# KaranSankla/Lidar_Object_Detection

Measured on AMD Instinct MI355X. Metric: LiDAR points/sec projected+instance-labelled, higher is better.
Workload: dtype f64

## Files before the change

### lidar_object_detection_amd/_build.py

```python
import hashlib
import os
import shutil
import subprocess

_HERE = os.path.dirname(os.path.abspath(__file__))
CSRC = os.path.join(_HERE, "csrc")
LIB = os.path.join(_HERE, "liblpf.so")
LAB_LIB = os.path.join(_HERE, "liblpf_lab.so")
SOURCES = ("lpf_api.hip", "lpf_kernels.hip.h", "lpf_reader.hip.h", "lpf_wide.hip.h", "lpf_cams.hip.h", "lpf_cams_wide.hip.h",
           "lpf_frame_wide.hip.h", "lpf_depth_maps.hip.h", "lpf_depth_overlays.hip.h",
           "lpf_match2d.hip.h", "lpf_inside.hip.h", "lpf_box_points.hip.h", "lpf_box_views.hip.h", "lpf_assign.hip.h",
           "lpf_first_match.hip.h", "lpf_rle.hip.h")
ARCH = "gfx950"

FLAGS = ["--offload-arch=" + ARCH, "-O3", "-std=c++17", "-fPIC", "-shared", "-pthread", "-ldl",
         "-ffp-contract=off", "-fno-fast-math", "-Wall", "-Wno-unused-function"]


def hipcc():
    exe = shutil.which("hipcc") or "/opt/rocm/bin/hipcc"
    if not os.path.exists(exe):
        raise RuntimeError("hipcc not found (looked on PATH and in /opt/rocm/bin)")
    return exe


HEADER = os.path.join(os.path.dirname(_HERE), "include", "lpf.h")
_MARKER = b"LPF_BUILD_ID="


def source_id(lab=False):
    h = hashlib.sha256()
    for path in [os.path.join(CSRC, s) for s in SOURCES] + [HEADER]:
# ... 67 lines not shown
```

### lidar_object_detection_amd/csrc/lpf_api.hip

```cpp
#include "lpf_kernels.hip.h"
#include "lpf_wide.hip.h"
#include "lpf_cams.hip.h"
#include "lpf_cams_wide.hip.h"
#include "lpf_frame_wide.hip.h"
#include "lpf_depth_maps.hip.h"
#include "lpf_depth_overlays.hip.h"
#include "lpf_match2d.hip.h"
#include "lpf_assign.hip.h"
#include "lpf_inside.hip.h"
#include "lpf_box_points.hip.h"
#include "lpf_box_views.hip.h"
#include "lpf_first_match.hip.h"
#include "lpf_rle.hip.h"
#include "../../include/lpf.h"

#include <algorithm>
#include <cmath>
#include <cstdarg>
#include <cstdio>
#include <cstdlib>
#include <cstring>
#include <dlfcn.h>
#include <initializer_list>
#include <mutex>
// ... 258 lines not shown
    return fn(Flag<false>());
}

static_assert(LPF_RECT_FUSED_TILE == 1024, "LpfDirectRect tiles are instantiated for 1024 points only");
template <bool STEP, typename Fn> void with_tile_form(const TileSource &src, int rows, bool scan_tail, Fn &&fn)
{
    auto tail = [&](auto lt, auto rw) {
        if (STEP && scan_tail) fn(lt, rw, Flag<STEP>()); else fn(lt, rw, Flag<false>());
    };
    if (src.kind == TileSource::DIRECT_RECT) {
        if (!src.f32) fn(TypeTag<LpfDirectRect<uint8_t, 0>>(), Rows<4>(), Flag<false>());
        else fn(TypeTag<LpfDirectRect<float, 1>>(), Rows<4>(), Flag<false>());
    } else if (src.kind == TileSource::DIRECT) {
        with_rule(src.f32, src.rule, [&](auto kind) { tail(TypeTag<LpfDirect<typename decltype(kind)::elem, decltype(kind)::rule>>(), Rows<2>()); });
    } else {
        with_label(src.label_bytes, [&](auto lt) {
            if (rows == 2) tail(lt, Rows<2>());
            else if (STEP && rows == 8) tail(lt, Rows<STEP ? 8 : 4>());
            else tail(lt, Rows<4>());
        });
    }
}

hipError_t host_wait(lpf_ctx *c)
{
    ++c->stats[0];
    return hipStreamSynchronize(c->stream);
}

void launch_tail(hipStream_t st, const LpfParams &P, int ntail, bool pre)
{
    if (pre) hipLaunchKernelGGL((lpf_tail_t<true>), dim3((unsigned)ntail), dim3(LPF_BLOCK), 0, st, P);
    else hipLaunchKernelGGL((lpf_tail_t<false>), dim3((unsigned)ntail), dim3(LPF_BLOCK), 0, st, P);
}

void box_job_camera(LpfBoxJob &J, const double K[9], int W, int H)
{
    memcpy(J.K, K, sizeof J.K);
    J.W = W; J.H = H;
}

int box_job_blocks(const lpf_ctx::BoxSet &B) { return B.F * B.job.chunks; }

int launch_box_job(lpf_ctx *c, lpf_ctx::BoxSet &B, const double K[9], int W, int H)
{
    if (!B.take_job()) return LPF_OK;
// ... 45 lines not shown
    if (ride) {
        const lpf_ctx::Unpacked &U = c->masks.unpacked;
        J.masks = (const uint8_t *)U.masks; J.label = U.label; J.M = U.M; J.hw = (long long)c->H * c->W;
        J.rects = U.rects; J.W = c->W;
        J.total16 = (long long)U.F * (J.hw / 16);
        Y.npack = (int)((J.total16 + LPF_BLOCK - 1) / LPF_BLOCK);
    }
    const int nk1_pad = (Y.nk1 + 7) & ~7;
    Y.nper = (Y.ntail + 7) / 8;
    Y.kper = Y.nk1 > 0 ? 8 : 0;
    if (Y.nper > 0 && Y.nk1 > 0) {
        const long long k = ((long long)nk1_pad * LPF_TAIL_SPREAD_20THS / 20 / 8) / Y.nper;
        Y.kper = (int)(k < 1 ? 1 : k) * 8;
    }
    const long long rest = (long long)nk1_pad - (long long)Y.nper * Y.kper;
    Y.rest = (int)(rest > 0 ? rest : 0);
    const long long grid = (long long)Y.nfin8 + Y.nbox8 + Y.nrg8 + (long long)Y.nper * (Y.kper + 8) + Y.rest + Y.npack;
    if (grid > 0) {
        const dim3 gs((unsigned)grid);
        ++c->stats[3];
        if (boxes) ++c->stats[5];
        with_tile_form<true>(tiles, KP.tile_pts >> 8, Q.valid && Q.pre, [&](auto lt, auto rw, auto pr) {
            with_flag(boxes, [&](auto bx) {
                hipLaunchKernelGGL((lpf_step_t<decltype(rw)::value, LPF_K1_FLAGS, typename decltype(lt)::type, decltype(pr)::value, decltype(bx)::value>),
                                   gs, dim3(LPF_BLOCK), 0, c->stream, KP, QP, RP, Y, J, XJ, GJ);
            });
        });
        LPF_HIP(c, hipGetLastError());
    }
    if (after) LPF_HIP(c, hipEventRecord(after, c->stream));
    if (KK.valid && KK.pre && KK.P.nseg_total > 0) {
        hipLaunchKernelGGL(lpf_scan_segments, dim3(KK.P.F), dim3(LPF_BLOCK), 0, c->stream, KK.P);
        LPF_HIP(c, hipGetLastError());
    }
    return LPF_OK;
}

lpf_ctx::Pending pending_run(const LpfParams &P, bool pre, int ntail, int nk1, const TileSource &src)
{
    return lpf_ctx::Pending{true, P, pre, ntail, nk1, src};
}

int queue_step(lpf_ctx *c, const lpf_ctx::Pending *cur, lpf_ctx::BoxSet *XB, hipEvent_t after, const LpfRectJob *RG)
{
    lpf_ctx::Pipeline &PL = c->pipe;
    const bool wait = cur && PL.defer;
    const lpf_ctx::Pending K = (cur && !wait) ? *cur : PL.k1, Q = PL.tail, R = PL.fin;
    int rc_ = launch_step(c, K, Q, R, cur ? &cur->src : nullptr, XB, after, RG);
// ... 545 lines not shown
}

int pack_unpacked(lpf_ctx *c)
{
    lpf_ctx::Masks &MK = c->masks;
    const lpf_ctx::Unpacked &U = MK.unpacked;
    if (!U.valid) return LPF_OK;
    lpf_ctx::Scratch &S = c->sc[MK.set];
    void *cur = nullptr;
    int rc = pack_masks(c, S.label_a, S.label_b, c->W, c->H, c->stream, U.masks, U.f32, U.rule, MK.bytes, U.F, U.M, 0, &cur, U.rects);
    if (rc) return rc;
    MK.packed(MK.F, MK.M, cur, MK.bytes);
    MK.forget_unpacked();
    return LPF_OK;
}

int plan_tile_source(lpf_ctx *c, bool fused, bool small, bool sparse_frames, int M, TileSource &src)
{
    src = TileSource();
    int rc;
    const lpf_ctx::Masks &MK = c->masks;
    const lpf_ctx::Unpacked &U = MK.unpacked;
    const bool readable = U.valid && U.pipelined == fused && M > 0 && sparse_frames;
    if (readable && !small && U.rects && ((!U.f32 && U.rule == 0) || (U.f32 && U.rule == 1))) src.kind = TileSource::DIRECT_RECT;
    else if (readable && small) src.kind = TileSource::DIRECT;
    else {
        src.ride_pack = U.valid && U.pipelined && fused && U.can_ride && M > 0;
        if (!src.ride_pack && (rc = pack_unpacked(c))) return rc;
        if (M > 0) src.kind = TileSource::PACKED;
    }
    if (M > 0 && fused && MK.set != c->pipe.run_set(fused))
        return fail(c, LPF_ERR_STATE, "the masks were set for another scratch set: in the pipelined modes the label images rotate with the scratch sets -- call lpf_set_masks_* before every lpf_run* (and after switching modes)");
    if (src.reads_masks()) {
        src.f32 = U.f32; src.rule = U.rule; src.img = U.masks;
        src.rects = U.rects;
    } else if (M > 0) {
        src.img = MK.img;
    }
    if (M > 0 && !src.img) return fail(c, LPF_ERR_STATE, "no masks for this run's scratch set: in the pipelined modes the label images rotate with the scratch sets -- call lpf_set_masks_* before every lpf_run* (and after switching modes)");
    src.label_bytes = (M > 0) ? MK.bytes : 4;
    return LPF_OK;
}


int check_frames(lpf_ctx *c, const char *who, const float *pts, const int64_t *frame_off, int F, int64_t slack)
{
    if (frame_off[0] != 0) return fail(c, LPF_ERR_ARG, "%s: frame_off[0] must be 0", who);
// ... 35 lines not shown
            if ((rc = reserve(c, dr, (size_t)F * m.M * 16))) return rc;
            LPF_HIP(c, hipMemcpyAsync(dr.p, m.rects, (size_t)F * m.M * 16, hipMemcpyHostToDevice, c->stream));
            d_rects = (const int32_t *)dr.p;
        }
        *host_in = true;
    }
    *masks = d_masks;
    *rects = rects_hold(m) ? (const int4 *)d_rects : nullptr;
    return LPF_OK;
}

struct Cam {
    const double *T, *K;
    double dmin, dmax;
    int W, H;
};
Cam ctx_cam(const lpf_ctx *c) { return Cam{c->T, c->K, c->dmin, c->dmax, c->W, c->H}; }
Cam input_cam(const lpf_cam_input &I) { return Cam{I.T_velo_to_rect, I.K, I.depth_min_excl, I.depth_max_excl, I.W, I.H}; }
void set_cam(LpfCam &P, const Cam &k)
{
    memcpy(P.T, k.T, sizeof P.T);
    memcpy(P.K, k.K, sizeof P.K);
    P.dmin = k.dmin; P.dmax = k.dmax; P.W = k.W; P.H = k.H;
}

struct NarrowLayout {
    int F = 0;
    bool small = false;
    int64_t seg_pts = 0;
    int nseg_total = 0, ngrp_total = 0, max_ngrp = 0;
    int nblk = 0;
    int nwblk = 0;
    int csplit = 1, ncblk = 0;
    bool few = false;
    bool pre_scan = false;
    int nseg_cap() const { return nseg_total > 0 ? nseg_total : 1; }
    int ngrp_cap() const { return ngrp_total > 0 ? ngrp_total : 1; }
    void split(int parts) { csplit = parts; ncblk = nwblk * parts; }
};

void narrow_layout(lpf_ctx *c, const int64_t *frame_off, int F, const lpf_ctx::BoxSet &BX, long long inst_cap, bool small, NarrowLayout &L)
{
    L = NarrowLayout();
    L.F = F; L.small = small;
    L.seg_pts = small ? LPF_SEG_SMALL : LPF_SEG_QUANTUM;
    c->h_frames.resize(F);
// ... 719 lines not shown
            LPF_HIP(c, hipEventCreate(&b));
            c->ev.push_back(a); c->ev.push_back(b);
        }
        e0 = c->ev[2 * c->ev_used]; e1 = c->ev[2 * c->ev_used + 1];
        ++c->ev_used;
        LPF_HIP(c, hipEventRecord(e0, c->stream));
    }
    if (fused) {
        const lpf_ctx::Pending cur = pending_run(P, L.pre_scan, ntail, nk1, src);
        if ((rc = queue_step(c, &cur, &BX, e1, (rect_tiles && tiles_wait) ? &RG : nullptr))) return rc;
        c->masks.forget_unpacked();
        c->pipe.parity = (c->pipe.parity + 1) % c->pipe.sets();
        return LPF_OK;
    }
    if (BX.job_ready() && nk1 > 0) {
        const lpf_ctx::Pending cur = pending_run(P, false, 0, nk1, src);
        lpf_ctx::Pending none;
        if ((rc = launch_step(c, cur, none, none, nullptr, &BX, e1))) return rc;
    } else {
    if ((rc = launch_box_job(c, BX))) return rc;
    if (nk1 > 0) {
        const dim3 g1((unsigned)nk1);
        with_tile_form<false>(src, P.tile_pts >> 8, false, [&](auto lt, auto rw, auto) {
            hipLaunchKernelGGL((lpf_k1_project_t<decltype(rw)::value, LPF_K1_FLAGS, typename decltype(lt)::type>), g1, dim3(LPF_BLOCK), 0, c->stream, P);
        });
        LPF_HIP(c, hipGetLastError());
        if (e1) LPF_HIP(c, hipEventRecord(e1, c->stream));
    }
    }
    if (L.pre_scan && L.nseg_total > 0) {
        hipLaunchKernelGGL(lpf_scan_segments, dim3(F), dim3(LPF_BLOCK), 0, c->stream, P);
        LPF_HIP(c, hipGetLastError());
    }
    if (ntail > 0) {
        if (small && P.count_boxes && c->geometry != 4 && (L.nblk <= LPF_WIDE_BELOW || c->geometry == 1)) {
            if (L.pre_scan) hipLaunchKernelGGL((lpf_tail_wide_t<true>), dim3((unsigned)ntail), dim3(64 * LPF_WIDE_WAVES), 0, c->stream, P);
            else hipLaunchKernelGGL((lpf_tail_wide_t<false>), dim3((unsigned)ntail), dim3(64 * LPF_WIDE_WAVES), 0, c->stream, P);
        } else {
            launch_tail(c->stream, P, ntail, L.pre_scan);
        }
        LPF_HIP(c, hipGetLastError());
    }
    hipLaunchKernelGGL(lpf_finalize, dim3(F), dim3(LPF_BLOCK), 0, c->stream, P);
    LPF_HIP(c, hipGetLastError());

    if (host_io) {
        std::vector<lpf_frame_summary> hs((size_t)F);
// ... 1626 lines not shown
```

### lidar_object_detection_amd/csrc/lpf_cams.hip.h

```cpp
#pragma once
#include "lpf_kernels.hip.h"

#define LPF_MAX_CAMS_DEV 4

struct LpfCamsArgs {
    LpfParams P[LPF_MAX_CAMS_DEV];
    int C;
    int ntail[LPF_MAX_CAMS_DEV];
};
static_assert(sizeof(LpfCamsArgs) <= 4096, "a kernel's argument segment holds 4 KB");

template <int ROWS, typename LT>
__global__ __launch_bounds__(LPF_BLOCK) void lpf_cams_stream(const LpfCamsArgs A)
{
    __shared__ unsigned s_cnt[LPF_MAX_CAMS_DEV][LPF_TAB_ROWS];
    float4 p[ROWS];
    lpf_k1_tile<ROWS, LPF_K1_FLAGS, LT, false>(A.P[0], (int)blockIdx.x, s_cnt[0], p);
    for (int cam = 1; cam < A.C; ++cam)
        lpf_k1_tile<ROWS, LPF_K1_FLAGS, LT, true>(A.P[cam], (int)blockIdx.x, s_cnt[cam], p);
}

template <bool PRE>
__global__ __launch_bounds__(LPF_BLOCK, 7) void lpf_cams_tail(const LpfCamsArgs A)
{
    __shared__ __attribute__((aligned(16))) char s_raw[LPF_TAIL_LDS];
    const int cam = (int)blockIdx.y;
    if ((int)blockIdx.x >= A.ntail[cam]) return;
    lpf_tail_block<PRE, 1>(A.P[cam], (int)blockIdx.x, s_raw);
}

__global__ __launch_bounds__(LPF_BLOCK) void lpf_cams_finalize(const LpfCamsArgs A)
{
    __shared__ unsigned s_tot[LPF_TAB_ROWS], s_c[LPF_FIN_STAGE];
    const LpfParams &P = A.P[blockIdx.y];
    const int f = (int)blockIdx.x;
    const LpfFrame fr = lpf_frame_record(P.frame0, P.frames, P.F > 1, f);
    lpf_finalize_frame(P, fr, f, s_tot, s_c);
}
```

### lidar_object_detection_amd/csrc/lpf_kernels.hip.h

```cpp
#pragma once
#include <hip/hip_runtime.h>
#include <stdint.h>

#define LPF_BLOCK 256
#define LPF_SEG_QUANTUM 4096
#define LPF_SEG_SMALL 1024
#define LPF_GROUP_SEGS 64
#define LPF_FRM_SHARDS 8
#define LPF_MAX_MASKS_DEV 32
#define LPF_TAB_ROWS 36
#define LPF_TAB_GROUPS 9

struct LpfFrame {
    long long pt_off;
    long long inst_base;
    int N;
    int seg_off;
    int nseg;
    int box_off;
    int B;
    int pad;
    long long cand_off;
    int cand_words;
    int grp_off;
    int shift;
    int pad4;
};

struct LpfCam {
    double T[12];
    double K[9];
    double dmin, dmax;
    int W, H;
};

struct LpfParams : LpfCam {
    int F, M;
    int seg_pts;
    int nseg_total;
    int nseg_cap;
    int ngrp_cap;
    int oriented;
    long long inst_cap;
    LpfFrame frame0;
    const LpfFrame *frames;
    const LpfFrame *segs;
    const int2 *blks;
    const int4 *cblks;
    int nblk, ncblk;
    int lists_small;
    int csplit;
    const float4 *pts;
    const void *label_img;
    const int4 *rects;
    const uint32_t *rect_grid;
    int rg_cw, rg_cells;
    const double *boxp;
    const float *boxq;
    const unsigned long long *cand;
    int2 *uv;
    uint32_t *label_bits;
    double *depth, *uf, *vf;
    long long *valid_idx;
    int2 *uv_valid;
    uint32_t *label_valid;
    long long *inst_idx;
    int32_t *count_out;
    void *summary;
    unsigned long long *vbal, *mbal;
    uint4 *seg_tab;
    uint4 *grp_tab;
    uint4 *frm_tab;
    uint4 *seg_pre;
    unsigned *cnt;
    float4 *mlist;
    int count_boxes;
    int count_lazy;
    int tile_pts;
};
static_assert(sizeof(LpfCam) == 192 && sizeof(LpfParams) == 576, "the camera leads LpfParams; neither layout may move");

__device__ __forceinline__ int lpf_lane() { return threadIdx.x & 63; }
__device__ __forceinline__ int lpf_wave() { return threadIdx.x >> 6; }

__device__ __forceinline__ int lpf_xcd_remap(int b, int n)
{
    const int q = n >> 3, r = n & 7, x = b & 7, i = b >> 3;
    return (x < r ? x * (q + 1) : r * (q + 1) + (x - r) * q) + i;
}

__device__ __forceinline__ int lpf_uni(int v) { return __builtin_amdgcn_readfirstlane(v); }
__device__ __forceinline__ long long lpf_uni64(long long v)
{
    return (long long)(((unsigned long long)(unsigned)lpf_uni((int)((unsigned long long)v >> 32)) << 32) | (unsigned)lpf_uni((int)v));
}
__device__ __forceinline__ LpfFrame lpf_frame_record(const LpfFrame &by_value, const LpfFrame *table, const bool many, const int idx)
{
    LpfFrame fr = by_value;
    if (many) {
        const LpfFrame t = table[lpf_uni(idx)];
        fr.pt_off = lpf_uni64(t.pt_off); fr.inst_base = lpf_uni64(t.inst_base); fr.N = lpf_uni(t.N); fr.seg_off = lpf_uni(t.seg_off);
        fr.nseg = lpf_uni(t.nseg); fr.box_off = lpf_uni(t.box_off); fr.B = lpf_uni(t.B); fr.pad = lpf_uni(t.pad);
        fr.cand_off = lpf_uni64(t.cand_off); fr.cand_words = lpf_uni(t.cand_words); fr.grp_off = lpf_uni(t.grp_off); fr.shift = lpf_uni(t.shift);
    }
    return fr;
}

__device__ __forceinline__ int32_t lpf_sat_i32(double r)
{
    int v;
    asm("v_cvt_i32_f64 %0, %1" : "=v"(v) : "v"(r));
    return (r != r) ? INT32_MIN : v;
}

__device__ __forceinline__ unsigned lpf_expo(double x) { return ((unsigned)__double2hiint(x) >> 20) & 0x7ffu; }

__device__ __forceinline__ void lpf_div2(double qx, double qy, double ad, double &uf, double &vf)
{
    const unsigned ea = lpf_expo(ad), ex = lpf_expo(qx), ey = lpf_expo(qy);
    const unsigned lo = min(ea, min(ex, ey)), hi = max(ea, max(ex, ey));
    if (lo >= 723u && hi <= 1323u) {
        double r = __builtin_amdgcn_rcp(ad);
        double e = fma(-ad, r, 1.0); r = fma(r, e, r);
        e = fma(-ad, r, 1.0);        r = fma(r, e, r);
        double q = qx * r; double s = fma(-ad, q, qx); uf = fma(s, r, q);
        q = qy * r;        s = fma(-ad, q, qy);        vf = fma(s, r, q);
    } else {
        uf = qx / ad;
        vf = qy / ad;
    }
}

__device__ __forceinline__ void lpf_project_point(const LpfCam &P, float fx, float fy, float fz,
                                                  double &uf, double &vf, double &d)
{
    const double x = (double)fx, y = (double)fy, z = (double)fz;
    double cx = P.T[0] * x; cx = fma(P.T[1], y, cx); cx = fma(P.T[2],  z, cx); cx = cx + P.T[3];
    double cy = P.T[4] * x; cy = fma(P.T[5], y, cy); cy = fma(P.T[6],  z, cy); cy = cy + P.T[7];
    double cz = P.T[8] * x; cz = fma(P.T[9], y, cz); cz = fma(P.T[10], z, cz); cz = cz + P.T[11];
    double qx = P.K[0] * cx; qx = fma(P.K[1], cy, qx); qx = fma(P.K[2], cz, qx);
    double qy = P.K[3] * cx; qy = fma(P.K[4], cy, qy); qy = fma(P.K[5], cz, qy);
    d = P.K[6] * cx; d = fma(P.K[7], cy, d); d = fma(P.K[8], cz, d);
    if (d == 0.0) d = -1e-6;
    lpf_div2(qx, qy, fabs(d), uf, vf);
}

__device__ __forceinline__ bool lpf_in_view(const LpfCam &P, int ui, int vi, double d)
{
    return ((unsigned)ui < (unsigned)P.W) && ((unsigned)vi < (unsigned)P.H) && (d > P.dmin) && (d < P.dmax);
}

__device__ __forceinline__ bool lpf_pixel(const LpfCam &P, double uf, double vf, double d, int &ui, int &vi)
{
    ui = lpf_sat_i32(rint(uf));
    vi = lpf_sat_i32(rint(vf));
    return lpf_in_view(P, ui, vi, d);
}

__device__ __forceinline__ unsigned lpf_f32_to_u8(float v)
{
    int t;
    if (!(v > -2147483904.0f && v < 2147483648.0f)) t = INT32_MIN; else t = (int)v;
    return (unsigned)t & 0xFFu;
}

template <typename T, int MODE>
__device__ __forceinline__ bool lpf_member(T v)
{
    if (MODE == 0) return v != 0;
    if (MODE == 1) return lpf_f32_to_u8((float)v) != 0u;
    if (MODE == 3) return (float)v > 0.5f;
    return lpf_f32_to_u8((float)v * 255.0f) == 255u;
}

template <typename T, int MODE> struct LpfDirect { };
template <typename LT> struct LpfIsDirect { static constexpr bool value = false; };
template <typename T, int MODE> struct LpfIsDirect<LpfDirect<T, MODE> > { static constexpr bool value = true; };

template <typename T, int MODE> struct LpfDirectRect { };
// ... 34 lines not shown
        }
        return l;
    }
    static __device__ __forceinline__ size_t frame_stride(const LpfParams &P) { return (size_t)P.M * (size_t)P.W * (size_t)P.H; }
};

template <typename T, int MODE>
struct LpfLabelSrc<LpfDirectRect<T, MODE> > {
    typedef T elem;
    static constexpr int mode = MODE;
    static __device__ __forceinline__ uint32_t get(const elem *__restrict__, const LpfParams &, const int, const int4 *, int, int) { return 0u; }
    static __device__ __forceinline__ size_t frame_stride(const LpfParams &P) { return (size_t)P.M * (size_t)P.W * (size_t)P.H; }
};

#define LPF_F_X4 1u
#define LPF_F_NTLOAD 2u
#define LPF_F_NTSTORE 4u
#define LPF_F_LAB_NOMATH 8u
#define LPF_F_LAB_NOGATHER 16u
#define LPF_F_LAB_NOSTORE 32u

#define LPF_F_LAB_NOBAL 64u
#define LPF_F_LAB_NOTAB 128u

#define LPF_RG_SHIFT 4
#define LPF_RG_CELL (1 << LPF_RG_SHIFT)
__device__ __forceinline__ unsigned lpf_wave_or(unsigned x);

template <int ROWS, unsigned FL, typename LT, bool PRELOADED>
__device__ __forceinline__ void lpf_k1_tile(const LpfParams &P, const int blk, unsigned *s_cnt, float4 (&p)[ROWS])
{
    constexpr int TILE = LPF_BLOCK * ROWS;
    static_assert(LPF_SEG_QUANTUM % TILE == 0 && (LPF_SEG_SMALL % TILE == 0 || ROWS >= 8), "tiles must divide segments (8-row and larger tiles: large geometry only)");
    const int tid = threadIdx.x, lane = lpf_lane(), wave = lpf_wave();
    const int tiles_per_seg = P.seg_pts / TILE;
    const int lb = lpf_xcd_remap(blk, P.nseg_total * tiles_per_seg);
    const int sid = lb / tiles_per_seg;
    LpfFrame fr = P.frame0;
    if (P.F > 1) fr = P.segs[__builtin_amdgcn_readfirstlane(sid)];
    const int f = fr.pad;
    const int sh = fr.shift;
    const long long pbase = fr.pt_off - sh;
    const int seg_start = (sid - fr.seg_off) * P.seg_pts;
    const int seg_end = min(seg_start + P.seg_pts, fr.N + sh);
    const int c = seg_start + (lb - sid * tiles_per_seg) * TILE;
    if (c >= seg_end) return;
    const float4 *__restrict__ pts = P.pts + pbase;
    typedef LpfLabelSrc<LT> Src;
    const typename Src::elem *__restrict__ limg =
        (P.label_img && P.M > 0) ? static_cast<const typename Src::elem *>(P.label_img) + (size_t)f * Src::frame_stride(P) : nullptr;
    const int rows_per_seg = P.seg_pts >> 6;
    if (tid < LPF_TAB_ROWS) s_cnt[tid] = 0;
    __syncthreads();
    unsigned nvalid_w = 0, nmask_w = 0;

    {
        const int wbase = c + wave * (ROWS * 64) + lane;
#pragma unroll
        for (int r = 0; r < ROWS; ++r) {
            if constexpr (PRELOADED) continue;
            const float4 *src = pts + min(wbase + r * 64, seg_end - 1);
            if (FL & LPF_F_NTLOAD) {
                typedef float f4v __attribute__((ext_vector_type(4)));
                const f4v t = __builtin_nontemporal_load(reinterpret_cast<const f4v *>(src));
                p[r] = make_float4(t.x, t.y, t.z, t.w);
            } else {
                p[r] = *src;
            }
        }
        uint32_t lab[ROWS];
        bool valid[ROWS];
        constexpr bool RECT = LpfIsDirectRect<LT>::value;
        const int4 *__restrict__ rc_f = ((RECT || LpfIsDirect<LT>::value) && P.rects) ? P.rects + (size_t)f * P.M : nullptr;
        const uint32_t *__restrict__ rgrid = (RECT && limg && P.rect_grid) ? P.rect_grid + (size_t)f * P.rg_cells : nullptr;
        const size_t mhw = (size_t)P.W * (size_t)P.H;
        unsigned long long myv = 0, mym = 0;
        auto consume = [&](const int r, uint32_t l, const bool okr) {
            const int idx = wbase + r * 64;
            if (idx >= sh && idx < seg_end && P.label_bits && !(FL & LPF_F_LAB_NOSTORE)) {
                if (FL & LPF_F_NTSTORE) __builtin_nontemporal_store(l, P.label_bits + pbase + idx);
                else P.label_bits[pbase + idx] = l;
            }
            const unsigned long long vb = __ballot(okr);
            const unsigned long long mb = __ballot(l != 0);
            if (lane == r) { myv = vb; mym = mb; }
            if (l && P.mlist && !(FL & LPF_F_LAB_NOSTORE))
                P.mlist[pbase + (wbase - lane) + ((wbase - lane) == 0 ? sh : 0) + nmask_w + __popcll(mb & ((1ull << lane) - 1ull))] =
                    make_float4(p[r].x, p[r].y, p[r].z, __uint_as_float(l));
            nvalid_w += __popcll(vb);
            nmask_w += __popcll(mb);
            while (l) {
                const int m = __ffs(l) - 1;
                l &= l - 1;
                atomicAdd(&s_cnt[2 + m], 1u);
            }
        };
#pragma unroll
        for (int r = 0; r < ROWS; ++r) {
            const int idx = wbase + r * 64;
            const bool live = idx >= sh && idx < seg_end;
            if (FL & LPF_F_X4) asm volatile("" ::"v"(p[r].w));
            double uf, vf, d, ru, rv;
            if (FL & LPF_F_LAB_NOMATH) {
                uf = (double)p[r].x; vf = (double)p[r].y; d = (double)p[r].z;
                ru = uf + 700.0; rv = vf + 100.0;
            } else {
                lpf_project_point(P, p[r].x, p[r].y, p[r].z, uf, vf, d);
                ru = rint(uf); rv = rint(vf);
            }
            const int ui = lpf_sat_i32(ru), vi = lpf_sat_i32(rv);
            const bool ok = live && ((unsigned)ui < (unsigned)P.W) && ((unsigned)vi < (unsigned)P.H) &&
                            (d > P.dmin) && (d < P.dmax);
            valid[r] = ok;
            lab[r] = 0;
            if constexpr (RECT) {
                if (ok && rgrid) lab[r] = rgrid[(vi >> LPF_RG_SHIFT) * P.rg_cw + (ui >> LPF_RG_SHIFT)];
            } else
            if (!(FL & LPF_F_LAB_NOGATHER)) {
                if (ok && limg) lab[r] = Src::get(limg, P, vi * P.W + ui, rc_f, ui, vi);
            }
            if (live && !(FL & LPF_F_LAB_NOSTORE)) {
                const long long g = pbase + idx;
                if (P.uv) {
                    if (FL & LPF_F_NTSTORE) {
                        typedef int i2v __attribute__((ext_vector_type(2)));
                        i2v t; t.x = ui; t.y = vi;
                        __builtin_nontemporal_store(t, reinterpret_cast<i2v *>(P.uv + g));
                    } else {
                        P.uv[g] = make_int2(ui, vi);
                    }
                }
                if (P.depth) P.depth[g] = d;
                if (P.uf) P.uf[g] = uf;
                if (P.vf) P.vf[g] = vf;
            }
        }
#pragma unroll
        for (int r = 0; r < ROWS; ++r) {
            uint32_t l = lab[r];
            if constexpr (RECT) {
                if (__any(l != 0u)) {
                    double uf, vf, d;
                    lpf_project_point(P, p[r].x, p[r].y, p[r].z, uf, vf, d);
                    const int ui = lpf_sat_i32(rint(uf)), vi = lpf_sat_i32(rint(vf));
                    const unsigned pix = (unsigned)(vi * P.W + ui);
                    uint32_t any = lpf_wave_or(l), l2 = 0u;
                    while (any) {
                        const int m = __ffs(any) - 1;
                        any &= any - 1u;
                        const int4 q = rc_f[m];
                        const bool in = ((l >> m) & 1u) && ui >= q.x && ui < q.z && vi >= q.y && vi < q.w;
                        if (__any(in)) {
                            const typename Src::elem *__restrict__ mk = limg + (size_t)m * mhw;
                            if (in && lpf_member<typename Src::elem, Src::mode>(mk[pix])) l2 |= 1u << m;
                        }
                    }
                    l = l2;
                }
            }
            consume(r, l, valid[r]);
        }
        if (lane < ROWS && !(FL & LPF_F_LAB_NOBAL)) {
            const size_t row = (size_t)sid * rows_per_seg + ((c - seg_start) >> 6) + wave * ROWS + lane;
            P.vbal[row] = myv;
            P.mbal[row] = mym;
        }
    }
    if (lane == 0) { atomicAdd(&s_cnt[0], nvalid_w); atomicAdd(&s_cnt[1], nmask_w); }
    __syncthreads();
    if (!(FL & LPF_F_LAB_NOTAB)) {
        if (tid < (2 + P.M + 1) >> 1) {
            const unsigned long long v = (unsigned long long)s_cnt[2 * tid] | ((unsigned long long)s_cnt[2 * tid + 1] << 32);
            if (v) {
                int seg_off = P.frame0.seg_off, grp_off = P.frame0.grp_off, fid = P.frame0.pad;
                if (P.F > 1) { const LpfFrame *e = P.segs + lpf_uni(sid); seg_off = e->seg_off; grp_off = e->grp_off; fid = e->pad; }
                const int k = sid - seg_off, g = tid >> 1, h = tid & 1;
                atomicAdd(reinterpret_cast<unsigned long long *>(P.seg_tab + (size_t)g * P.nseg_cap + sid) + h, v);
                atomicAdd(reinterpret_cast<unsigned long long *>(P.grp_tab + (size_t)g * P.ngrp_cap + grp_off + (k >> 6)) + h, v);
                atomicAdd(reinterpret_cast<unsigned long long *>(P.frm_tab + ((size_t)fid * LPF_FRM_SHARDS + (k & (LPF_FRM_SHARDS - 1))) * LPF_TAB_GROUPS + g) + h, v);
            }
        }
    }
}

template <int ROWS, unsigned FL, typename LT>
__device__ __forceinline__ void lpf_k1_tile(const LpfParams &P, const int blk, unsigned *s_cnt)
{
    float4 p[ROWS];
// ... 906 lines not shown
    int F, M, cw, ch, cells, bpf;
};
__device__ __forceinline__ void lpf_rect_grid_block(const LpfRectJob &G, const int blk)
{
    const int f = blk / G.bpf, i = (blk - f * G.bpf) * LPF_BLOCK + (int)threadIdx.x;
    if (f >= G.F || i >= G.cells) return;
    const int cy = i / G.cw, cx = i - cy * G.cw;
    const int x0 = cx << LPF_RG_SHIFT, y0 = cy << LPF_RG_SHIFT;
    const int4 *__restrict__ rc = G.rects + (size_t)lpf_uni(f) * G.M;
    uint32_t bits = 0u;
    for (int m0 = 0; m0 < G.M; m0 += 8) {
        int4 q[8];
#pragma unroll
        for (int j = 0; j < 8; ++j) q[j] = rc[min(m0 + j, G.M - 1)];
#pragma unroll
        for (int j = 0; j < 8; ++j)
            if (m0 + j < G.M && q[j].x < x0 + LPF_RG_CELL && q[j].z > x0 && q[j].y < y0 + LPF_RG_CELL && q[j].w > y0 && q[j].z > q[j].x && q[j].w > q[j].y)
                bits |= 1u << (m0 + j);
    }
    G.grid[(size_t)f * G.cells + i] = bits;
}
__global__ __launch_bounds__(LPF_BLOCK) void lpf_rect_grid_kernel(const LpfRectJob G) { lpf_rect_grid_block(G, (int)blockIdx.x); }

template <int ROWS, unsigned FL, typename LT, bool PRE, bool BOXES>
__global__ __launch_bounds__(LPF_BLOCK, 7) void lpf_step_t(const LpfParams P, const LpfParams Q, const LpfParams R, const LpfStepLayout Y,
                                                           const LpfPackJob J, const LpfBoxJob X, const LpfRectJob G)
{
    __shared__ __attribute__((aligned(16))) char s_raw[LPF_STEP_LDS];
    __shared__ unsigned s_cnt[LPF_TAB_ROWS];
    int b = (int)blockIdx.x;
    LPF_ROLE_BEGIN
    if (b < Y.nfin8) {
        if (b < Y.nfin) {
            const LpfFrame fr = lpf_frame_record(R.frame0, R.frames, R.F > 1, b);
            lpf_finalize_frame(R, fr, b, s_cnt, reinterpret_cast<unsigned *>(s_raw));
            LPF_ROLE_END(0)
        }
        return;
    }
    b -= Y.nfin8;
    if (b < Y.nbox8) {
        if constexpr (BOXES) {
            if (b < Y.nbox) { lpf_box_frame_block(X, b, s_raw); LPF_ROLE_END(1) }
        }
        return;
    }
// ... 680 lines not shown
```

Before: 173.1 billion.

## Fold K·T into one matrix with certified fast projection and exact fallback

Precomputes the combined 3x4 projection matrix K·T and error bounds on the host. The per-point path then uses a single affine transform and one Newton-refined reciprocal, and falls back to the exact two-stage projection with full division only when a wave contains a point near a rounding or depth boundary. It also stops writing float depth/uv outputs through a template flag, caches the packed pixel index instead of reprojecting points in the rect path, and replaces per-lane ballot storage with writelane ops. The gain comes from much less f64 arithmetic per point, in exchange for a larger kernel argument struct and a subtle error-bound argument that must stay correct.

New measurement: 174.0 billion, median of 6. Within noise of the previous version (+0.6%).

```diff
diff --git a/lidar_object_detection_amd/_build.py b/lidar_object_detection_amd/_build.py
--- a/lidar_object_detection_amd/_build.py
+++ b/lidar_object_detection_amd/_build.py
@@ -7,7 +7,7 @@
 CSRC = os.path.join(_HERE, "csrc")
 LIB = os.path.join(_HERE, "liblpf.so")
 LAB_LIB = os.path.join(_HERE, "liblpf_lab.so")
-SOURCES = ("lpf_api.hip", "lpf_kernels.hip.h", "lpf_reader.hip.h", "lpf_wide.hip.h", "lpf_cams.hip.h", "lpf_cams_wide.hip.h",
+SOURCES = ("lpf_api.hip", "lpf_kernels.hip.h", "lpf_project.hip.h", "lpf_reader.hip.h", "lpf_wide.hip.h", "lpf_cams.hip.h", "lpf_cams_wide.hip.h",
            "lpf_frame_wide.hip.h", "lpf_depth_maps.hip.h", "lpf_depth_overlays.hip.h",
            "lpf_match2d.hip.h", "lpf_inside.hip.h", "lpf_box_points.hip.h", "lpf_box_views.hip.h", "lpf_assign.hip.h",
            "lpf_first_match.hip.h", "lpf_rle.hip.h")
diff --git a/lidar_object_detection_amd/csrc/lpf_api.hip b/lidar_object_detection_amd/csrc/lpf_api.hip
--- a/lidar_object_detection_amd/csrc/lpf_api.hip
+++ b/lidar_object_detection_amd/csrc/lpf_api.hip
@@ -304,6 +304,8 @@
     }
 }
 
+bool tile_fvals(const LpfParams &P) { return P.depth || P.uf || P.vf; }
+
 hipError_t host_wait(lpf_ctx *c)
 {
     ++c->stats[0];
@@ -395,8 +397,11 @@
         if (boxes) ++c->stats[5];
         with_tile_form<true>(tiles, KP.tile_pts >> 8, Q.valid && Q.pre, [&](auto lt, auto rw, auto pr) {
             with_flag(boxes, [&](auto bx) {
-                hipLaunchKernelGGL((lpf_step_t<decltype(rw)::value, LPF_K1_FLAGS, typename decltype(lt)::type, decltype(pr)::value, decltype(bx)::value>),
-                                   gs, dim3(LPF_BLOCK), 0, c->stream, KP, QP, RP, Y, J, XJ, GJ);
+                with_flag(tile_fvals(KP), [&](auto fv) {
+                    hipLaunchKernelGGL((lpf_step_t<decltype(rw)::value, LPF_K1_FLAGS | (decltype(fv)::value ? LPF_F_FVALS : 0u), typename decltype(lt)::type,
+                                                   decltype(pr)::value, decltype(bx)::value>),
+                                       gs, dim3(LPF_BLOCK), 0, c->stream, KP, QP, RP, Y, J, XJ, GJ);
+                });
             });
         });
         LPF_HIP(c, hipGetLastError());
@@ -988,7 +993,8 @@
     const lpf_ctx::Masks &MK = c->masks;
     const lpf_ctx::Unpacked &U = MK.unpacked;
     const bool readable = U.valid && U.pipelined == fused && M > 0 && sparse_frames;
-    if (readable && !small && U.rects && ((!U.f32 && U.rule == 0) || (U.f32 && U.rule == 1))) src.kind = TileSource::DIRECT_RECT;
+    const bool pix16 = c->W <= 65535 && c->H <= 65535;
+    if (readable && !small && pix16 && U.rects && ((!U.f32 && U.rule == 0) || (U.f32 && U.rule == 1))) src.kind = TileSource::DIRECT_RECT;
     else if (readable && small) src.kind = TileSource::DIRECT;
     else {
         src.ride_pack = U.valid && U.pipelined && fused && U.can_ride && M > 0;
@@ -1070,6 +1076,7 @@
     memcpy(P.T, k.T, sizeof P.T);
     memcpy(P.K, k.K, sizeof P.K);
     P.dmin = k.dmin; P.dmax = k.dmax; P.W = k.W; P.H = k.H;
+    lpf_cam_prepare(P);
 }
 
 struct NarrowLayout {
@@ -1835,7 +1842,10 @@
     if (nk1 > 0) {
         const dim3 g1((unsigned)nk1);
         with_tile_form<false>(src, P.tile_pts >> 8, false, [&](auto lt, auto rw, auto) {
-            hipLaunchKernelGGL((lpf_k1_project_t<decltype(rw)::value, LPF_K1_FLAGS, typename decltype(lt)::type>), g1, dim3(LPF_BLOCK), 0, c->stream, P);
+            with_flag(tile_fvals(P), [&](auto fv) {
+                hipLaunchKernelGGL((lpf_k1_project_t<decltype(rw)::value, LPF_K1_FLAGS | (decltype(fv)::value ? LPF_F_FVALS : 0u), typename decltype(lt)::type>),
+                                   g1, dim3(LPF_BLOCK), 0, c->stream, P);
+            });
         });
         LPF_HIP(c, hipGetLastError());
         if (e1) LPF_HIP(c, hipEventRecord(e1, c->stream));
diff --git a/lidar_object_detection_amd/csrc/lpf_cams.hip.h b/lidar_object_detection_amd/csrc/lpf_cams.hip.h
--- a/lidar_object_detection_amd/csrc/lpf_cams.hip.h
+++ b/lidar_object_detection_amd/csrc/lpf_cams.hip.h
@@ -15,9 +15,10 @@
 {
     __shared__ unsigned s_cnt[LPF_MAX_CAMS_DEV][LPF_TAB_ROWS];
     float4 p[ROWS];
-    lpf_k1_tile<ROWS, LPF_K1_FLAGS, LT, false>(A.P[0], (int)blockIdx.x, s_cnt[0], p);
+    constexpr unsigned FL = LPF_K1_FLAGS | LPF_F_FVALS;
+    lpf_k1_tile<ROWS, FL, LT, false>(A.P[0], (int)blockIdx.x, s_cnt[0], p);
     for (int cam = 1; cam < A.C; ++cam)
-        lpf_k1_tile<ROWS, LPF_K1_FLAGS, LT, true>(A.P[cam], (int)blockIdx.x, s_cnt[cam], p);
+        lpf_k1_tile<ROWS, FL, LT, true>(A.P[cam], (int)blockIdx.x, s_cnt[cam], p);
 }
 
 template <bool PRE>
diff --git a/lidar_object_detection_amd/csrc/lpf_kernels.hip.h b/lidar_object_detection_amd/csrc/lpf_kernels.hip.h
--- a/lidar_object_detection_amd/csrc/lpf_kernels.hip.h
+++ b/lidar_object_detection_amd/csrc/lpf_kernels.hip.h
@@ -1,6 +1,7 @@
 #pragma once
 #include <hip/hip_runtime.h>
 #include <stdint.h>
+#include "lpf_project.hip.h"
 
 #define LPF_BLOCK 256
 #define LPF_SEG_QUANTUM 4096
@@ -25,13 +26,6 @@
     int grp_off;
     int shift;
     int pad4;
-};
-
-struct LpfCam {
-    double T[12];
-    double K[9];
-    double dmin, dmax;
-    int W, H;
 };
 
 struct LpfParams : LpfCam {
@@ -78,7 +72,7 @@
     int count_lazy;
     int tile_pts;
 };
-static_assert(sizeof(LpfCam) == 192 && sizeof(LpfParams) == 576, "the camera leads LpfParams; neither layout may move");
+static_assert(sizeof(LpfCam) == 344 && sizeof(LpfParams) == 728, "the camera leads LpfParams; neither layout may move");
 
 __device__ __forceinline__ int lpf_lane() { return threadIdx.x & 63; }
 __device__ __forceinline__ int lpf_wave() { return threadIdx.x >> 6; }
@@ -104,57 +98,6 @@
         fr.cand_off = lpf_uni64(t.cand_off); fr.cand_words = lpf_uni(t.cand_words); fr.grp_off = lpf_uni(t.grp_off); fr.shift = lpf_uni(t.shift);
     }
     return fr;
-}
-
-__device__ __forceinline__ int32_t lpf_sat_i32(double r)
-{
-    int v;
-    asm("v_cvt_i32_f64 %0, %1" : "=v"(v) : "v"(r));
-    return (r != r) ? INT32_MIN : v;
-}
-
-__device__ __forceinline__ unsigned lpf_expo(double x) { return ((unsigned)__double2hiint(x) >> 20) & 0x7ffu; }
-
-__device__ __forceinline__ void lpf_div2(double qx, double qy, double ad, double &uf, double &vf)
-{
-    const unsigned ea = lpf_expo(ad), ex = lpf_expo(qx), ey = lpf_expo(qy);
-    const unsigned lo = min(ea, min(ex, ey)), hi = max(ea, max(ex, ey));
-    if (lo >= 723u && hi <= 1323u) {
-        double r = __builtin_amdgcn_rcp(ad);
-        double e = fma(-ad, r, 1.0); r = fma(r, e, r);
-        e = fma(-ad, r, 1.0);        r = fma(r, e, r);
-        double q = qx * r; double s = fma(-ad, q, qx); uf = fma(s, r, q);
-        q = qy * r;        s = fma(-ad, q, qy);        vf = fma(s, r, q);
-    } else {
-        uf = qx / ad;
-        vf = qy / ad;
-    }
-}
-
-__device__ __forceinline__ void lpf_project_point(const LpfCam &P, float fx, float fy, float fz,
-                                                  double &uf, double &vf, double &d)
-{
-    const double x = (double)fx, y = (double)fy, z = (double)fz;
-    double cx = P.T[0] * x; cx = fma(P.T[1], y, cx); cx = fma(P.T[2],  z, cx); cx = cx + P.T[3];
-    double cy = P.T[4] * x; cy = fma(P.T[5], y, cy); cy = fma(P.T[6],  z, cy); cy = cy + P.T[7];
-    double cz = P.T[8] * x; cz = fma(P.T[9], y, cz); cz = fma(P.T[10], z, cz); cz = cz + P.T[11];
-    double qx = P.K[0] * cx; qx = fma(P.K[1], cy, qx); qx = fma(P.K[2], cz, qx);
-    double qy = P.K[3] * cx; qy = fma(P.K[4], cy, qy); qy = fma(P.K[5], cz, qy);
-    d = P.K[6] * cx; d = fma(P.K[7], cy, d); d = fma(P.K[8], cz, d);
-    if (d == 0.0) d = -1e-6;
-    lpf_div2(qx, qy, fabs(d), uf, vf);
-}
-
-__device__ __forceinline__ bool lpf_in_view(const LpfCam &P, int ui, int vi, double d)
-{
-    return ((unsigned)ui < (unsigned)P.W) && ((unsigned)vi < (unsigned)P.H) && (d > P.dmin) && (d < P.dmax);
-}
-
-__device__ __forceinline__ bool lpf_pixel(const LpfCam &P, double uf, double vf, double d, int &ui, int &vi)
-{
-    ui = lpf_sat_i32(rint(uf));
-    vi = lpf_sat_i32(rint(vf));
-    return lpf_in_view(P, ui, vi, d);
 }
 
 __device__ __forceinline__ unsigned lpf_f32_to_u8(float v)
@@ -235,10 +178,24 @@
 
 #define LPF_F_LAB_NOBAL 64u
 #define LPF_F_LAB_NOTAB 128u
-
+#define LPF_F_FVALS 256u
+
+#ifndef LPF_LEAN_ROWS
+#define LPF_LEAN_ROWS 8
+#endif
 #define LPF_RG_SHIFT 4
 #define LPF_RG_CELL (1 << LPF_RG_SHIFT)
 __device__ __forceinline__ unsigned lpf_wave_or(unsigned x);
+__device__ __forceinline__ void lpf_set_lane64(int &lo, int &hi, unsigned long long s, int l)
+{
+    const unsigned s0 = (unsigned)s, s1 = (unsigned)(s >> 32);
+    switch (l) {
+#define LPF_SET_LANE(i) case i: asm("s_nop 1\n\tv_writelane_b32 %0, %2, " #i "\n\tv_writelane_b32 %1, %3, " #i : "+v"(lo), "+v"(hi) : "s"(s0), "s"(s1)); break;
+        LPF_SET_LANE(0) LPF_SET_LANE(1) LPF_SET_LANE(2) LPF_SET_LANE(3) LPF_SET_LANE(4) LPF_SET_LANE(5) LPF_SET_LANE(6) LPF_SET_LANE(7)
+        LPF_SET_LANE(8) LPF_SET_LANE(9) LPF_SET_LANE(10) LPF_SET_LANE(11) LPF_SET_LANE(12) LPF_SET_LANE(13) LPF_SET_LANE(14) LPF_SET_LANE(15)
+#undef LPF_SET_LANE
+    }
+}
 
 template <int ROWS, unsigned FL, typename LT, bool PRELOADED>
 __device__ __forceinline__ void lpf_k1_tile(const LpfParams &P, const int blk, unsigned *s_cnt, float4 (&p)[ROWS])
@@ -268,7 +225,8 @@
     unsigned nvalid_w = 0, nmask_w = 0;
 
     {
-        const int wbase = c + wave * (ROWS * 64) + lane;
+        const int wfirst = lpf_uni(c + wave * (ROWS * 64));
+        const int wbase = wfirst + lane;
 #pragma unroll
         for (int r = 0; r < ROWS; ++r) {
             if constexpr (PRELOADED) continue;
@@ -282,25 +240,23 @@
             }
         }
         uint32_t lab[ROWS];
-        bool valid[ROWS];
         constexpr bool RECT = LpfIsDirectRect<LT>::value;
+        unsigned pix[RECT ? ROWS : 1];
         const int4 *__restrict__ rc_f = ((RECT || LpfIsDirect<LT>::value) && P.rects) ? P.rects + (size_t)f * P.M : nullptr;
         const uint32_t *__restrict__ rgrid = (RECT && limg && P.rect_grid) ? P.rect_grid + (size_t)f * P.rg_cells : nullptr;
         const size_t mhw = (size_t)P.W * (size_t)P.H;
-        unsigned long long myv = 0, mym = 0;
-        auto consume = [&](const int r, uint32_t l, const bool okr) {
+        int myv_lo = 0, myv_hi = 0, mym_lo = 0, mym_hi = 0;
+        auto consume = [&](const int r, uint32_t l) {
             const int idx = wbase + r * 64;
-            if (idx >= sh && idx < seg_end && P.label_bits && !(FL & LPF_F_LAB_NOSTORE)) {
+            if (wbase >= sh - r * 64 && wbase < seg_end - r * 64 && P.label_bits && !(FL & LPF_F_LAB_NOSTORE)) {
                 if (FL & LPF_F_NTSTORE) __builtin_nontemporal_store(l, P.label_bits + pbase + idx);
                 else P.label_bits[pbase + idx] = l;
             }
-            const unsigned long long vb = __ballot(okr);
-            const unsigned long long mb = __ballot(l != 0);
-            if (lane == r) { myv = vb; mym = mb; }
+            const unsigned long long mb = __builtin_amdgcn_ballot_w64(l != 0);
+            lpf_set_lane64(mym_lo, mym_hi, mb, r);
             if (l && P.mlist && !(FL & LPF_F_LAB_NOSTORE))
-                P.mlist[pbase + (wbase - lane) + ((wbase - lane) == 0 ? sh : 0) + nmask_w + __popcll(mb & ((1ull << lane) - 1ull))] =
+                P.mlist[pbase + wfirst + (wfirst == 0 ? sh : 0) + nmask_w + __popcll(mb & ((1ull << lane) - 1ull))] =
                     make_float4(p[r].x, p[r].y, p[r].z, __uint_as_float(l));
-            nvalid_w += __popcll(vb);
             nmask_w += __popcll(mb);
             while (l) {
                 const int m = __ffs(l) - 1;
@@ -311,20 +267,39 @@
 #pragma unroll
         for (int r = 0; r < ROWS; ++r) {
             const int idx = wbase + r * 64;
-            const bool live = idx >= sh && idx < seg_end;
+            const bool live = wbase >= sh - r * 64 && wbase < seg_end - r * 64;
             if (FL & LPF_F_X4) asm volatile("" ::"v"(p[r].w));
-            double uf, vf, d, ru, rv;
-            if (FL & LPF_F_LAB_NOMATH) {
-                uf = (double)p[r].x; vf = (double)p[r].y; d = (double)p[r].z;
-                ru = uf + 700.0; rv = vf + 100.0;
+            double uf = 0.0, vf = 0.0, d = 0.0;
+            int ui, vi;
+            bool ok;
+            if constexpr ((FL & (LPF_F_FVALS | LPF_F_LAB_NOMATH)) != 0u) {
+                double ru, rv;
+                if (FL & LPF_F_LAB_NOMATH) {
+                    uf = (double)p[r].x; vf = (double)p[r].y; d = (double)p[r].z;
+                    ru = uf + 700.0; rv = vf + 100.0;
+                } else {
+                    lpf_project_point(P, p[r].x, p[r].y, p[r].z, uf, vf, d);
+                    ru = rint(uf); rv = rint(vf);
+                }
+                ui = lpf_sat_i32(ru); vi = lpf_sat_i32(rv);
+                ok = live && ((unsigned)ui < (unsigned)P.W) && ((unsigned)vi < (unsigned)P.H) && (d > P.dmin) && (d < P.dmax);
             } else {
-                lpf_project_point(P, p[r].x, p[r].y, p[r].z, uf, vf, d);
-                ru = rint(uf); rv = rint(vf);
-            }
-            const int ui = lpf_sat_i32(ru), vi = lpf_sat_i32(rv);
-            const bool ok = live && ((unsigned)ui < (unsigned)P.W) && ((unsigned)vi < (unsigned)P.H) &&
-                            (d > P.dmin) && (d < P.dmax);
-            valid[r] = ok;
+                bool in_view;
+                const bool sure = lpf_pixel_fast<(ROWS >= LPF_LEAN_ROWS)>(P, p[r].x, p[r].y, p[r].z, ui, vi, in_view);
+                const unsigned long long unsure = __builtin_amdgcn_ballot_w64(live & !sure);
+                if (lpf_uni((int)((unsigned)unsure | (unsigned)(unsure >> 32))) != 0) {
+                    int z = 0;
+                    float cx = p[r].x, cy = p[r].y, cz = p[r].z;
+                    asm volatile("" : "+s"(z), "+v"(cx), "+v"(cy), "+v"(cz));
+                    in_view = lpf_pixel_exact(P, P.T + z, P.K + z, cx, cy, cz, ui, vi);
+                }
+                ok = live && in_view;
+            }
+            {
+                const unsigned long long vb = __builtin_amdgcn_ballot_w64(ok);
+                lpf_set_lane64(myv_lo, myv_hi, vb, r);
+                nvalid_w += __popcll(vb);
+            }
             lab[r] = 0;
             if constexpr (RECT) {
                 if (ok && rgrid) lab[r] = rgrid[(vi >> LPF_RG_SHIFT) * P.rg_cw + (ui >> LPF_RG_SHIFT)];
@@ -343,20 +318,21 @@
                         P.uv[g] = make_int2(ui, vi);
                     }
                 }
-                if (P.depth) P.depth[g] = d;
-                if (P.uf) P.uf[g] = uf;
-                if (P.vf) P.vf[g] = vf;
-            }
+                if constexpr ((FL & LPF_F_FVALS) != 0u) {
+                    if (P.depth) P.depth[g] = d;
+                    if (P.uf) P.uf[g] = uf;
+                    if (P.vf) P.vf[g] = vf;
+                }
+            }
+            if constexpr (RECT) pix[r] = (unsigned)ui | ((unsigned)vi << 16);
         }
 #pragma unroll
         for (int r = 0; r < ROWS; ++r) {
             uint32_t l = lab[r];
             if constexpr (RECT) {
                 if (__any(l != 0u)) {
-                    double uf, vf, d;
-                    lpf_project_point(P, p[r].x, p[r].y, p[r].z, uf, vf, d);
-                    const int ui = lpf_sat_i32(rint(uf)), vi = lpf_sat_i32(rint(vf));
-                    const unsigned pix = (unsigned)(vi * P.W + ui);
+                    const int ui = (int)(pix[r] & 0xffffu), vi = (int)(pix[r] >> 16);
+                    const unsigned pixel = (unsigned)(vi * P.W + ui);
                     uint32_t any = lpf_wave_or(l), l2 = 0u;
                     while (any) {
                         const int m = __ffs(any) - 1;
@@ -365,18 +341,18 @@
                         const bool in = ((l >> m) & 1u) && ui >= q.x && ui < q.z && vi >= q.y && vi < q.w;
                         if (__any(in)) {
                             const typename Src::elem *__restrict__ mk = limg + (size_t)m * mhw;
-                            if (in && lpf_member<typename Src::elem, Src::mode>(mk[pix])) l2 |= 1u << m;
+                            if (in && lpf_member<typename Src::elem, Src::mode>(mk[pixel])) l2 |= 1u << m;
                         }
                     }
                     l = l2;
                 }
             }
-            consume(r, l, valid[r]);
+            consume(r, l);
         }
         if (lane < ROWS && !(FL & LPF_F_LAB_NOBAL)) {
             const size_t row = (size_t)sid * rows_per_seg + ((c - seg_start) >> 6) + wave * ROWS + lane;
-            P.vbal[row] = myv;
-            P.mbal[row] = mym;
+            P.vbal[row] = (unsigned long long)(unsigned)myv_lo | ((unsigned long long)(unsigned)myv_hi << 32);
+            P.mbal[row] = (unsigned long long)(unsigned)mym_lo | ((unsigned long long)(unsigned)mym_hi << 32);
         }
     }
     if (lane == 0) { atomicAdd(&s_cnt[0], nvalid_w); atomicAdd(&s_cnt[1], nmask_w); }
@@ -1329,6 +1305,8 @@
 }
 __global__ __launch_bounds__(LPF_BLOCK) void lpf_rect_grid_kernel(const LpfRectJob G) { lpf_rect_grid_block(G, (int)blockIdx.x); }
 
+static_assert(3 * sizeof(LpfParams) + sizeof(LpfStepLayout) + sizeof(LpfPackJob) + sizeof(LpfBoxJob) + sizeof(LpfRectJob) + 64 <= 4096,
+              "lpf_step_t's arguments (three runs by value) must fit the 4 KB argument segment");
 template <int ROWS, unsigned FL, typename LT, bool PRE, bool BOXES>
 __global__ __launch_bounds__(LPF_BLOCK, 7) void lpf_step_t(const LpfParams P, const LpfParams Q, const LpfParams R, const LpfStepLayout Y,
                                                            const LpfPackJob J, const LpfBoxJob X, const LpfRectJob G)
diff --git a/lidar_object_detection_amd/csrc/lpf_project.hip.h b/lidar_object_detection_amd/csrc/lpf_project.hip.h
--- /dev/null
+++ b/lidar_object_detection_amd/csrc/lpf_project.hip.h
@@ -0,0 +1,183 @@
+#pragma once
+#include <math.h>
+#include <stdint.h>
+#include <string.h>
+
+#if defined(__HIPCC__)
+#include <hip/hip_runtime.h>
+#define LPF_PD __device__ __forceinline__
+#else
+#define LPF_PD static inline
+#endif
+#ifndef LPF_RCP
+#define LPF_RCP(x) __builtin_amdgcn_rcp(x)
+#endif
+
+struct LpfCam {
+    double T[12];
+    double K[9];
+    double dmin, dmax;
+    int W, H;
+    double M[12];
+    double eq, ed;
+    double d_in_lo, d_in_hi;
+    double d_out_lo, d_out_hi;
+    float amax;
+    int pad;
+};
+static_assert(sizeof(LpfCam) == 344, "LpfCam travels by value in kernel arguments: move its layout deliberately");
+
+#define LPF_FAST_AMAX 128.0f
+#define LPF_FAST_TAU 0x1p-43
+
+static inline void lpf_cam_prepare(LpfCam &C)
+{
+    double G = 0.0, Gd = 0.0, kmax = 0.0;
+    for (int i = 0; i < 3; ++i) {
+        double g = 0.0;
+        for (int j = 0; j < 4; ++j) {
+            double m = 0.0, a = 0.0;
+            for (int k = 0; k < 3; ++k) { m += C.K[3 * i + k] * C.T[4 * k + j]; a += fabs(C.K[3 * i + k]) * fabs(C.T[4 * k + j]); }
+            C.M[4 * i + j] = m;
+            g += a;
+        }
+        G = fmax(G, g);
+        Gd = g;
+        for (int k = 0; k < 3; ++k) kmax = fmax(kmax, fabs(C.K[3 * i + k]));
+    }
+    bool finite = true;
+    for (int i = 0; i < 12; ++i) finite = finite && isfinite(C.M[i]) && isfinite(C.T[i]);
+    for (int i = 0; i < 9; ++i) finite = finite && isfinite(C.K[i]);
+    const bool ok = finite && Gd >= 0x1p-100 && G <= 0x1p500 && kmax <= 0x1p100;
+    C.eq = 0x1p-48 * (G * (1.0 + 0x1p-40));
+    C.ed = 0x1p-48 * (Gd * (1.0 + 0x1p-40));
+    const double E = C.ed * (double)LPF_FAST_AMAX;
+    C.amax = ok ? LPF_FAST_AMAX : 0.0f;
+    C.pad = 0;
+    C.d_in_lo = nextafter(C.dmin + E, INFINITY);
+    C.d_in_hi = nextafter(C.dmax - E, -INFINITY);
+    C.d_out_lo = nextafter(C.dmin - E, -INFINITY);
+    C.d_out_hi = nextafter(C.dmax + E, INFINITY);
+}
+
+#if defined(__HIP_DEVICE_COMPILE__)
+LPF_PD int32_t lpf_cvt_i32(double r)
+{
+    int v;
+    asm("v_cvt_i32_f64 %0, %1" : "=v"(v) : "v"(r));
+    return v;
+}
+LPF_PD unsigned lpf_hi32(double x) { return (unsigned)__double2hiint(x); }
+#else
+LPF_PD int32_t lpf_cvt_i32(double r)
+{
+    if (r != r) return 0;
+    if (r >= 2147483648.0) return INT32_MAX;
+    if (r <= -2147483648.0) return INT32_MIN;
+    return (int32_t)r;
+}
+LPF_PD unsigned lpf_hi32(double x) { uint64_t b; memcpy(&b, &x, 8); return (unsigned)(b >> 32); }
+#endif
+LPF_PD int32_t lpf_sat_i32(double r) { return (r != r) ? INT32_MIN : lpf_cvt_i32(r); }
+
+LPF_PD unsigned lpf_expo(double x) { return (lpf_hi32(x) >> 20) & 0x7ffu; }
+
+LPF_PD void lpf_div2(double qx, double qy, double ad, double &uf, double &vf)
+{
+#if defined(__HIP_DEVICE_COMPILE__)
+    const unsigned ea = lpf_expo(ad), ex = lpf_expo(qx), ey = lpf_expo(qy);
+    const unsigned lo = min(ea, min(ex, ey)), hi = max(ea, max(ex, ey));
+    if (lo >= 723u && hi <= 1323u) {
+        double r = __builtin_amdgcn_rcp(ad);
+        double e = fma(-ad, r, 1.0); r = fma(r, e, r);
+        e = fma(-ad, r, 1.0);        r = fma(r, e, r);
+        double q = qx * r; double s = fma(-ad, q, qx); uf = fma(s, r, q);
+        q = qy * r;        s = fma(-ad, q, qy);        vf = fma(s, r, q);
+    } else
+#endif
+    {
+        uf = qx / ad;
+        vf = qy / ad;
+    }
+}
+
+LPF_PD void lpf_project_point(const double *T, const double *K, float fx, float fy, float fz, double &uf, double &vf, double &d)
+{
+    const double x = (double)fx, y = (double)fy, z = (double)fz;
+    double cx = T[0] * x; cx = fma(T[1], y, cx); cx = fma(T[2],  z, cx); cx = cx + T[3];
+    double cy = T[4] * x; cy = fma(T[5], y, cy); cy = fma(T[6],  z, cy); cy = cy + T[7];
+    double cz = T[8] * x; cz = fma(T[9], y, cz); cz = fma(T[10], z, cz); cz = cz + T[11];
+    double qx = K[0] * cx; qx = fma(K[1], cy, qx); qx = fma(K[2], cz, qx);
+    double qy = K[3] * cx; qy = fma(K[4], cy, qy); qy = fma(K[5], cz, qy);
+    d = K[6] * cx; d = fma(K[7], cy, d); d = fma(K[8], cz, d);
+    if (d == 0.0) d = -1e-6;
+    lpf_div2(qx, qy, fabs(d), uf, vf);
+}
+LPF_PD void lpf_project_point(const LpfCam &P, float fx, float fy, float fz, double &uf, double &vf, double &d)
+{
+    lpf_project_point(P.T, P.K, fx, fy, fz, uf, vf, d);
+}
+
+LPF_PD bool lpf_in_view(const LpfCam &P, int ui, int vi, double d)
+{
+    return ((unsigned)ui < (unsigned)P.W) && ((unsigned)vi < (unsigned)P.H) && (d > P.dmin) && (d < P.dmax);
+}
+
+LPF_PD bool lpf_pixel(const LpfCam &P, double uf, double vf, double d, int &ui, int &vi)
+{
+    ui = lpf_sat_i32(rint(uf));
+    vi = lpf_sat_i32(rint(vf));
+    return lpf_in_view(P, ui, vi, d);
+}
+
+LPF_PD bool lpf_pixel_exact(const LpfCam &P, const double *T, const double *K, float fx, float fy, float fz, int &ui, int &vi)
+{
+    const double x = (double)fx, y = (double)fy, z = (double)fz;
+    double cx = T[0] * x; cx = fma(T[1], y, cx); cx = fma(T[2],  z, cx); cx = cx + T[3];
+    double cy = T[4] * x; cy = fma(T[5], y, cy); cy = fma(T[6],  z, cy); cy = cy + T[7];
+    double cz = T[8] * x; cz = fma(T[9], y, cz); cz = fma(T[10], z, cz); cz = cz + T[11];
+    double qx = K[0] * cx; qx = fma(K[1], cy, qx); qx = fma(K[2], cz, qx);
+    double qy = K[3] * cx; qy = fma(K[4], cy, qy); qy = fma(K[5], cz, qy);
+    double d = K[6] * cx; d = fma(K[7], cy, d); d = fma(K[8], cz, d);
+    if (d == 0.0) d = -1e-6;
+    double ad = fabs(d);
+    ui = lpf_sat_i32(rint(qx / ad));
+#if defined(__HIP_DEVICE_COMPILE__)
+    asm volatile("" : "+v"(ad) : "v"(ui));
+#endif
+    vi = lpf_sat_i32(rint(qy / ad));
+    return lpf_in_view(P, ui, vi, d);
+}
+
+template <bool LEAN = false>
+LPF_PD bool lpf_pixel_fast(const LpfCam &P, float fx, float fy, float fz, int &ui, int &vi, bool &in_view)
+{
+    const double x = (double)fx, y = (double)fy, z = (double)fz;
+    double qx, qy, d;
+    if (LEAN) {
+        qx = fma(P.M[0], x, fma(P.M[1], y, P.M[2]  * z)) + P.M[3];
+        qy = fma(P.M[4], x, fma(P.M[5], y, P.M[6]  * z)) + P.M[7];
+        d  = fma(P.M[8], x, fma(P.M[9], y, P.M[10] * z)) + P.M[11];
+    } else {
+        qx = fma(P.M[0], x, fma(P.M[1], y, fma(P.M[2],  z, P.M[3])));
+        qy = fma(P.M[4], x, fma(P.M[5], y, fma(P.M[6],  z, P.M[7])));
+        d  = fma(P.M[8], x, fma(P.M[9], y, fma(P.M[10], z, P.M[11])));
+    }
+    const double a = fabs(d);
+    double r = LPF_RCP(a);
+    const double e = fma(-a, r, 1.0);
+    r = fma(r, e, r);
+    const double u = qx * r, v = qy * r;
+    const double ru = rint(u), rv = rint(v);
+    ui = lpf_cvt_i32(ru);
+    vi = lpf_cvt_i32(rv);
+    const float am = fmaxf(fmaxf(fabsf(fx), fabsf(fy)), fabsf(fz));
+    const double ar = fma((double)am, r, r);
+    const double td = fma(P.ed, ar, LPF_FAST_TAU), tq = P.eq * ar;
+    const double du = u - ru, dv = v - rv;
+    const double hu = fma(td, fabs(u), fabs(du)), hv = fma(td, fabs(v), fabs(dv));
+    const double lim = 0.5 - tq;
+    const bool d_in = (d > P.d_in_lo) & (d < P.d_in_hi);
+    in_view = ((unsigned)ui < (unsigned)P.W) & ((unsigned)vi < (unsigned)P.H) & d_in;
+    return (hu < lim) & (hv < lim) & (am < P.amax) & (d_in | (d < P.d_out_lo) | (d > P.d_out_hi));
+}
```
